# yahoo0742/COSNet

Measured on AMD Instinct MI355X. Metric: frame-pairs/sec (fwd+bwd) at 473x473 RGBD, higher is better.
Workload: dtype bf16; 1 GPU; RGBDSegmentation_RAA train step (fwd+loss+bwd+SGD), 473x473, batch 4 pairs/GPU; model=RGBDSegmentation_RAA(Bottleneck,[3,4,23,3],[3,4,6,3],1), global_batch=4, parallelism=dp1

## Files before the change

### cosnet_amd/_native.py

```python
import ctypes
import os

import torch

_HERE = os.path.dirname(os.path.abspath(__file__))
LIB_PATH = os.environ.get("COSNET_HIP_LIB") or os.path.join(_HERE, "_lib", "libcosnet_hip.so")

DT_F32 = 0
DT_BF16 = 1

_P = ctypes.c_void_p
_I = ctypes.c_int
_L = ctypes.c_longlong
_F = ctypes.c_float
_S = ctypes.c_size_t

_SIGS = {
    "cn_conv_fwd": (_I, [_I, _P, _L, _I, _I, _I, _I, _P, _I, _I, _I, _I, _I, _I, _P, _P, _L, _I, _I, _P]),
    "cn_conv_fwd_ws": (_I, [_I, _P, _L, _I, _I, _I, _I, _P, _I, _I, _I, _I, _I, _I, _P, _P, _L, _I, _I,
                            _P, _S, _P]),
    "cn_conv_fwd_workspace_floats": (_S, [_I, _I, _I, _I]),
    "cn_conv_dgrad": (_I, [_I, _P, _L, _I, _I, _I, _I, _P, _I, _I, _I, _I, _I, _I, _P, _L, _I, _I, _I, _P]),
    "cn_conv_wgrad_workspace_floats": (_S, [_I, _I, _I, _I, _I, _I, _I, _I]),
    "cn_conv_wgrad": (_I, [_I, _P, _L, _I, _I, _I, _I, _P, _L, _I, _I, _I, _I, _I, _I, _I, _I, _P, _P, _P]),
# ... 66 lines not shown
    "cn_avgpool": (_I, [_I, _P, _L, _I, _I, _I, _F, _P, _P, _P]),
    "cn_avgpool_workspace_floats": (_S, [_I, _I, _I, _I]),
    "cn_bcast_rows": (_I, [_I, _P, _I, _I, _I, _F, _P, _L, _I, _P]),
    "cn_gate_fwd": (_I, [_I, _P, _L, _I, _I, _P, _P, _P, _L, _P, _P]),
    "cn_gate_bwd": (_I, [_I, _P, _L, _P, _L, _P, _I, _I, _P, _I, _P, _L, _P, _P, _P, _P]),
    "cn_colpart_workspace_floats": (_S, [_I, _I]),
    "cn_mean_rows": (_I, [_P, _I, _I, _P, _P]),
    "cn_sum_rows": (_I, [_P, _I, _I, _P, _P]),
    "cn_scale_dev": (_I, [_P, _L, _P, _P, _P]),
    "cn_scale": (_I, [_P, _L, _F, _P]),
    "cn_soft_iou": (_I, [_P, _P, _I, _L, _P, _P, _P, _P]),
    "cn_frame_resize": (_I, [_I, _P, _I, _L, _L, _L, _I, _I, _I, _I, _P, _P, _I, _I, _I, _I, _P]),
    "cn_gemm_force_config": (_I, [_I]),
    "cn_gemm_ws_mode": (_I, [_I]),
    "cn_gemm_ws_launches": (_S, []),
    "cn_gemm_set_wgrad_target": (_I, [_I]),
    "cn_coatt_force_variant": (_I, [_I]),
    "cn_head_fwd": (_I, [_I, _P, _L, _P, _L, _I, _I, _I, _P, _P, _P, _L, _P, _P]),
    "cn_head_bwd": (_I, [_I, _P, _L, _P, _I, _I, _I, _P, _P, _L, _P, _P, _P, _P]),
    "cn_upsample_sigmoid": (_I, [_P, _I, _I, _I, _I, _I, _I, _P, _P]),
    "cn_upsample_sigmoid_bwd": (_I, [_P, _P, _I, _I, _I, _I, _I, _I, _P, _P]),
    "cn_count_ge": (_I, [_P, _L, _F, _P, _P]),
    "cn_loss_workspace_floats": (_S, [_L]),
    "cn_bce_l1": (_I, [_P, _P, _L, _F, _F, _P, _P, _P, _P]),
    "cn_bce_l1_devcount": (_I, [_P, _P, _L, _P, ctypes.c_double, _F, _P, _P, _P, _P]),
    "cn_sgd": (_I, [_P, _I, _P, _F, _F, _P]),
    "cn_rowdot": (_I, [_I, _P, _L, _P, _L, _I, _I, _P, _P]),
    "cn_colsum": (_I, [_I, _P, _L, _I, _I, _P, _P, _P]),
    "cn_cast2d": (_I, [_I, _I, _P, _L, _I, _I, _P, _L, _I, _P]),
    "cn_build_source_hash": (ctypes.c_char_p, []),
# ... 17 lines not shown
    if not os.path.exists(LIB_PATH):
        raise NativeError("libcosnet_hip.so not built (%s); run __graft_entry__.build()" % LIB_PATH)
    lib = ctypes.CDLL(LIB_PATH, mode=ctypes.RTLD_GLOBAL)
    for name, (res, args) in _SIGS.items():
        if os.environ.get("COSNET_HIP_LIB") and not hasattr(lib, name):
            continue
        fn = getattr(lib, name)
        fn.restype = res
        fn.argtypes = args
    _lib = lib
    return lib


HASHED_SOURCES = ["gemm.hip", "gemm_ws.hip", "conv.hip", "bn.hip", "ew.hip", "coatt.hip", "coatt_fused.hip",
                  "coatt_q48.hip", "coatt_flash.hip", "coatt_f8.hip", "fp8.hip", "frames.hip", "eval.hip",
                  "common.h", "gemm.h", "gemm_dev.h", "coatt_fused.h", "../../include/cosnet_hip.h"]


def source_hash():
    import hashlib
    h = hashlib.sha256()
    for f in HASHED_SOURCES:
        with open(os.path.join(_HERE, "csrc", f), "rb") as fh:
            h.update(fh.read())
    return h.hexdigest()[:16]


def build_info():
    import hashlib
    lib_hash = load().cn_build_source_hash().decode()
    with open(LIB_PATH, "rb") as fh:
# ... 39 lines not shown
```

### cosnet_amd/csrc/bn.hip

```cpp
#include "common.h"
#include "../../include/cosnet_hip.h"

namespace {

constexpr int UNR = 4;
constexpr int SUNR = 8;

struct Layout {
  int CPR, CB, RPB;
};
template <class T> __host__ __device__ inline Layout layout_red(int C) {
  Layout l;
  l.CPR = C / VecOf<T>::N;
  l.CB = l.CPR < 32 ? l.CPR : 32;
  l.RPB = 256 / l.CB;
  return l;
}
template <class T> __host__ __device__ inline Layout layout_of(int C) {
  Layout l;
  l.CPR = C / VecOf<T>::N;
  l.CB = l.CPR < 256 ? l.CPR : 256;
  l.RPB = 256 / l.CB;
  return l;
}
// ... 161 lines not shown
    const double md = s1 / n;
    const double q = s2 - s1 * md > 0 ? s2 - s1 * md : 0.0;
    const double var = q / n;
    mean[seg * C + c] = (float)(K + md);
    invstd[seg * C + c] = (float)(1.0 / sqrt(var + (double)eps));
    if (run_mean) {
      const double unb = n > 1 ? q / (n - 1) : var;
      rm = (float)((1.0 - momentum) * rm + momentum * (K + md));
      rv = (float)((1.0 - momentum) * rv + momentum * unb);
    }
  }
  if (run_mean) { run_mean[c] = (float)rm; run_var[c] = (float)rv; }
}

template <int NSEG>
__global__ __launch_bounds__(256) void bn_tile_stats_finalize(const float* __restrict__ ws, long long plane,
                                                              int mtiles, int BM, int M, int seg_rows,
                                                              int C, float* mean, float* invstd,
                                                              float* run_mean, float* run_var,
                                                              float momentum, float eps) {
  const int c0 = blockIdx.x * FCH;
  const int ch = threadIdx.x % FCH, lane = threadIdx.x / FCH, c = c0 + ch;
  double d1[NSEG], d2[NSEG];
#pragma unroll
  for (int s = 0; s < NSEG; ++s) { d1[s] = 0.0; d2[s] = 0.0; }
  if (c < C) {
    for (int t = lane; t < mtiles; t += 256 / FCH) {
      const int r0 = t * BM, r1 = min(M, r0 + BM);
      const int sA = r0 / seg_rows;
      const int endA = min(r1, (sA + 1) * seg_rows);
      const double nA = endA - r0, nB = r1 - endA;
      const long long o = (long long)t * C + c;
      const double K = ws[o];
      const double a1 = ws[o + plane], a2 = ws[o + 2 * plane];
#pragma unroll
      for (int s = 0; s < NSEG; ++s) {
        if (s == sA) { d1[s] += nA * K + a1; d2[s] += a2 + 2.0 * K * a1 + nA * K * K; }
        if (s == sA + 1 && nB > 0) {
          const double b1 = ws[o + 3 * plane], b2 = ws[o + 4 * plane];
          d1[s] += nB * K + b1;
          d2[s] += b2 + 2.0 * K * b1 + nB * K * K;
        }
      }
    }
  }
  __shared__ double red[2 * NSEG][4][FCH];
  const int wave = threadIdx.x / 64;
#pragma unroll
  for (int s = 0; s < NSEG; ++s) {
#pragma unroll
    for (int o = FCH; o < 64; o <<= 1) {
      d1[s] += __shfl_xor(d1[s], o, 64);
      d2[s] += __shfl_xor(d2[s], o, 64);
    }
    if ((threadIdx.x & 63) < FCH) { red[2 * s][wave][ch] = d1[s]; red[2 * s + 1][wave][ch] = d2[s]; }
  }
  __syncthreads();
  if (threadIdx.x >= FCH || c >= C) return;
  double rm = 0, rv = 0;
  if (run_mean) { rm = run_mean[c]; rv = run_var[c]; }
// ... 1 lines not shown
  for (int s = 0; s < NSEG; ++s) {
    const double s1 = ((red[2 * s][0][ch] + red[2 * s][1][ch]) + red[2 * s][2][ch]) + red[2 * s][3][ch];
    const double s2 = ((red[2 * s + 1][0][ch] + red[2 * s + 1][1][ch]) + red[2 * s + 1][2][ch]) + red[2 * s + 1][3][ch];
    const double md = s1 / n;
    double var = s2 / n - md * md;
    if (var < 0) var = 0;
    mean[s * C + c] = (float)md;
    invstd[s * C + c] = (float)(1.0 / sqrt(var + (double)eps));
    if (run_mean) {
      const double unb = n > 1 ? var * n / (n - 1) : var;
      rm = (float)((1.0 - momentum) * rm + momentum * md);
      rv = (float)((1.0 - momentum) * rv + momentum * unb);
    }
  }
  if (run_mean) { run_mean[c] = (float)rm; run_var[c] = (float)rv; }
}

__global__ void bn_eval_params(const float* rm, const float* rv, int C, float eps, float* mean, float* invstd) {
  int c = blockIdx.x * blockDim.x + threadIdx.x;
  if (c >= C) return;
  mean[c] = rm[c];
  invstd[c] = 1.0f / sqrtf(rv[c] + eps);
}

__device__ __forceinline__ unsigned pack4_fp8_bn(float a, float b, float c, float d) {
  a = fminf(fmaxf(a, -448.f), 448.f);
  b = fminf(fmaxf(b, -448.f), 448.f);
  c = fminf(fmaxf(c, -448.f), 448.f);
  d = fminf(fmaxf(d, -448.f), 448.f);
  unsigned w = __builtin_amdgcn_cvt_pk_fp8_f32(a, b, 0, false);
// ... 390 lines not shown
  const int seg_rows = M / nseg;
  const dim3 fin((C + FCH - 1) / FCH);
#define CN_TF(NS)                                                                                    \
  hipLaunchKernelGGL((bn_tile_stats_finalize<NS>), fin, dim3(256), 0, st, ws, plane, mtiles, BM, M, \
                     seg_rows, C, mean, invstd, run_mean, run_var, momentum, eps)
  switch (nseg) {
    case 1: CN_TF(1); break;
    case 2: CN_TF(2); break;
    default: return CN_ERR_UNSUPPORTED;
  }
#undef CN_TF
  CN_CHECK_LAUNCH();
  return 0;
}

int cn_bn_tile_bwd_impl(const float* ws, int mtiles, int C, float* sum_dz, float* sum_dzxh,
                        hipStream_t st) {
  const dim3 fin((C + FCH - 1) / FCH);
  hipLaunchKernelGGL(bn_bwd_finalize<2>, fin, dim3(256), 0, st, ws, mtiles, C, sum_dz, sum_dzxh,
                     (float*)nullptr);
  CN_CHECK_LAUNCH();
  return 0;
}

extern "C" int cn_bn_bwd_apply(int dtype, const void* x, long long ldx, const void* dy, long long lddy,
                               int P, int C, const float* mean, const float* invstd,
                               const float* gamma, const float* beta, const float* sum_dz,
                               const float* sum_dzxh, void* dx, long long lddx, hipStream_t st) {
  return with_dtype(dtype, [&](auto tag) {
    using T = tag_t<decltype(tag)>;
// ... 135 lines not shown
```

### cosnet_amd/csrc/conv.hip

```cpp
#include "gemm.h"
#include "../../include/cosnet_hip.h"

static GemmArgs gemm_defaults() {
  GemmArgs a = {};
  a.nsplit = 1;
  a.k_chunk = 1 << 30;
  a.alpha = 1.f;
  a.cfg = -1;
  FastDiv one = fastdiv_make(1);
  a.ga.div_C = a.ga.div_KW = a.ga.div_OW = a.ga.div_OHW = one;
  a.gb = a.ga;
  a.rm_div_OW = a.rm_div_OHW = one;
  return a;
}

static ConvGeom make_geom(int N, int H, int W, int C, int OH, int OW, int KH, int KW, int st,
                          int off_y, int off_x, int step_y, int step_x) {
  ConvGeom g;
  g.N = N; g.H = H; g.W = W; g.C = C; g.OH = OH; g.OW = OW; g.KH = KH; g.KW = KW; g.st = st;
  g.off_y = off_y; g.off_x = off_x; g.step_y = step_y; g.step_x = step_x;
  g.div_C = fastdiv_make(C);
  g.div_KW = fastdiv_make(KW);
  g.div_OW = fastdiv_make(OW);
  g.div_OHW = fastdiv_make(OH * OW);
// ... 193 lines not shown
  if (!fp8_operands_ok(Cout, lddy, dy8, wt8)) return CN_ERR_ALIGN;
  if (lddx % 8 || misaligned(dx)) return CN_ERR_ALIGN;
  GemmArgs a;
  int la;
  int rc = conv_dgrad_args(dy8, lddy, N, OH, OW, Cout, wt8, Cin, KH, KW, pad, dil, dx, lddx, H, W,
                           accumulate, true, a, la);
  if (rc) return rc;
  a.scale_a = dy_state;
  a.scale_b = w_state;
  return cn_gemm_dispatch(a, DT_FP8_E5M2, 0, la, L_KC_DENSE, 1, st);
}

int cn_bn_tile_stats_impl(const float* ws, long long plane, int mtiles, int BM, int M, int nseg, int C,
                          float* mean, float* invstd, float* run_mean, float* run_var, float momentum,
                          float eps, hipStream_t st);
int cn_bn_tile_bwd_impl(const float* ws, int mtiles, int C, float* sum_dz, float* sum_dzxh,
                        hipStream_t st);

static long long mtiles_of(int dtype, int M, int N, int K) {
  const int bm = cn_gemm_bm(dtype, M, N, K, -1);
  return (M + bm - 1) / bm;
}

extern "C" size_t cn_conv_fwd_bn_workspace_floats(int dtype, int M, int Cout, int K) {
  return (size_t)5 * mtiles_of(dtype, M, Cout, K) * Cout;
}

static int gemm_bn_stats(GemmArgs& a, int dtype, int la, int G, int nseg, float* const* ws,
                         float* const* mean, float* const* invstd, float* const* run_mean,
                         float* const* run_var, float momentum, float eps, hipStream_t st) {
  const int bm = cn_gemm_bm(dtype, a.M, a.N, a.K, -1);
  const long long mt = (a.M + bm - 1) / bm;
  a.st_mode = 1;
  a.st_ws = ws[0];
  a.st_plane = mt * a.N;
  a.st_seg_rows = a.M / nseg;
  int rc = cn_gemm_dispatch(a, dtype, 0, la, L_KC_DENSE, G, st);
  for (int g = 0; g < G && !rc; ++g)
    rc = cn_bn_tile_stats_impl(ws[g], a.st_plane, (int)mt, bm, a.M, nseg, a.N, mean[g], invstd[g],
                               run_mean[g], run_var[g], momentum, eps, st);
  return rc;
}

extern "C" int cn_conv_fwd_bn(int dtype, const void* x, long long ldx, int N, int H, int W, int Cin,
                              const void* w, int Cout, int KH, int KW, int stride, int pad, int dil,
                              const float* bias, void* y, long long ldy, int OH, int OW, int nseg,
                              float* ws, float* mean, float* invstd, float* run_mean, float* run_var,
                              float momentum, float eps, hipStream_t st) {
  GemmArgs a;
  int la;
  int rc = conv_fwd_args(dtype, x, ldx, N, H, W, Cin, w, Cout, KH, KW, stride, pad, dil, bias, y,
// ... 369 lines not shown
```

### cosnet_amd/csrc/gemm.h

```cpp
#pragma once
#include "common.h"

enum LoadKind { L_KC_DENSE = 0, L_KC_CONV = 1, L_MC_DENSE = 2, L_MC_CONV = 3,
                L_KC_CONV_G = 4 };

struct ConvGeom {
  int N, H, W, C;
  int OH, OW;
  int KH, KW;
  int st;
  int off_y, off_x, step_y, step_x;
  FastDiv div_C, div_KW, div_OW, div_OHW;
};

constexpr int GEMM_MAXG = 24;
struct GemmGroup {
  const void* A[GEMM_MAXG];
  const void* B[GEMM_MAXG];
  void* C[GEMM_MAXG];
  const float* SA[GEMM_MAXG];
  const float* SB[GEMM_MAXG];
  const float* bias[GEMM_MAXG];
  float* ST[GEMM_MAXG];
  int dil[GEMM_MAXG];
// ... 22 lines not shown
  long long st_plane;
  int st_seg_rows;
  const void* br_x; long long br_ldx;
  const float* br_mean; const float* br_invstd; const float* br_gamma; const float* br_beta;
  int ngroup;
  GemmGroup grp;
  int wt;
};

int cn_gemm_dispatch(const GemmArgs& a, int dtype, int c_f32, int la, int lb, int batch, hipStream_t st);
int cn_gemm_pick(int M, int N, int K, int batch_splits);
long long cn_gemm_cfg_blocks(int cfg, int M, int N);
int cn_gemm_bm(int dtype, int M, int N, int K, int cfg_or_minus1);
bool cn_gemm_ws_supports(const GemmArgs& a);
int cn_gemm_ws_launch(const GemmArgs& a, int walkers_per_xcd, hipStream_t st);
int cn_splitk_reduce_impl(const float* ws, int nsplit, long long slab, long long n, float* out,
                          int accumulate, hipStream_t st);
```

### cosnet_amd/csrc/gemm.hip

```cpp
#include "common.h"
#include "gemm.h"
#include "gemm_dev.h"
#include "../../include/cosnet_hip.h"

#include <type_traits>

namespace {

template <class T> struct Frag;
template <> struct Frag<bf16> { typedef bf16x8 type; };
template <> struct Frag<float> { typedef f32x4 type; };

__device__ __forceinline__ int mc_swz(int k, int granules_per_row) {
  int h = (k & 3) | (((k >> 3) & 1) << 2);
  return (granules_per_row >= 32 ? h : (h & 3)) << 2;
}

__device__ __forceinline__ int mc_swz8(int k) { return (k & 7) ^ ((k >> 5) & 1); }

__device__ __attribute__((aligned(16))) unsigned g_zero16[4];

__device__ __forceinline__ void glds16(const void* src, char* lds_wave_base) {
  __builtin_amdgcn_global_load_lds((const __attribute__((address_space(1))) void*)src,
                                   (__attribute__((address_space(3))) void*)lds_wave_base, 16, 0, 0);
// ... 1013 lines not shown
  return launch_c<f8e5m2, float, 11, L_MC_DENSE, LB>(a, batch, st);
}

static bool buf_ok(int kind, const GemmArgs& a, bool is_a, int esz) {
  const long long ld = is_a ? a.lda : a.ldb;
  const ConvGeom& g = is_a ? a.ga : a.gb;
  const long long kspan = a.nsplit > 1 ? a.k_chunk : a.K;
  if (kind == L_KC_DENSE) return 256 * ld * esz < 0x80000000ll && (long long)a.K * esz < 0xFFFF0000ll;
  if (kind == L_KC_CONV) return (long long)g.N * g.H * g.W * ld * esz < 0x80000000ll;
  if (kind == L_MC_DENSE) return (kspan + 128) * ld * esz < 0xFFFF0000ll && 128 * ld * esz < 0x80000000ll;
  return true;
}

static int g_ws_mode = 1;
static size_t g_ws_launches = 0;
static bool ws_heuristic(const GemmArgs& a) {
  return a.K <= 256 && a.N >= 4 * a.K && a.M >= 8192;
}
static bool ws_eligible(const GemmArgs& a, int dtype, int c_f32, int la, int lb, int batch) {
  if (!g_ws_mode || g_force_cfg >= 0 || a.cfg >= 0) return false;
  if (dtype != DT_BF16 || c_f32 || la != L_KC_DENSE || lb != L_KC_DENSE) return false;
  if (batch != 1 || a.nsplit != 1 || a.row_map || a.ngroup || a.st_mode) return false;
  if ((a.c_mode != 0 && a.c_mode != 2) || a.bias || a.alpha != 1.f || a.scale_a || a.scale_b) return false;
  if (!cn_gemm_ws_supports(a)) return false;
  return g_ws_mode >= 2 || ws_heuristic(a);
}

int cn_gemm_dispatch(const GemmArgs& a_in, int dtype, int c_f32, int la, int lb, int batch, hipStream_t st) {
  GemmArgs a = a_in;
  a.wt = a.c_mode != 1 && a.c_mode != 3 ? 4 : 0;
  if (a.M <= 0 || a.N <= 0 || batch <= 0) return 0;
  const int esz = (dtype == DT_FP8 || dtype == DT_FP8_E5M2) ? 1 : dtype == DT_BF16 ? 2 : 4;
  const int bk = 128 / esz;
  if (la == L_KC_CONV && (a.ga.C % bk != 0 || !buf_ok(L_KC_CONV, a, true, esz))) la = L_KC_CONV_G;
  if (!buf_ok(la, a, true, esz) || !buf_ok(lb, a, false, esz)) return CN_ERR_SHAPE;
  if (ws_eligible(a, dtype, c_f32, la, lb, batch)) {
    ++g_ws_launches;
    return cn_gemm_ws_launch(a, g_ws_mode == 3 ? 1 : 0, st);
  }
  if (dtype == DT_FP8) {
// ... 136 lines not shown
```

### cosnet_amd/csrc/gemm_ws.hip

```cpp
#include "common.h"
#include "gemm.h"
#include "gemm_dev.h"
#include "../../include/cosnet_hip.h"

#include <algorithm>
#include <cstdlib>
#include <type_traits>

namespace {

struct WsArgs {
  int M, N;
  const bf16* A; long long lda;
  const bf16* B; long long ldb;
  bf16* C; long long ldc;
  int nslices;
  int wpx;
  int wt;
};

__device__ __forceinline__ u32x4 load16_asm(const void* p) {
  u32x4 v;
  asm volatile("global_load_dwordx4 %0, %1, off" : "=&v"(v) : "v"(p) : "memory");
  return v;
}

template <int KEEP, bool TIE, int N>
__device__ __forceinline__ void wait_keep(u32x4 (&x)[N]) {
  static_assert(KEEP < 64, "vmcnt is 6 bits");
  asm volatile("s_waitcnt vmcnt(%0)" :: "n"(KEEP) : "memory");
  if constexpr (TIE) {
#pragma unroll
    for (int i = 0; i < N; ++i) asm volatile("" : "+v"(x[i]));
  }
}

template <int KT, int BM, int BN, int WM, int WN, bool MODE2, bool BREG>
__global__ __launch_bounds__(WM * WN * 64, 1) void gemm_ws_kernel(WsArgs p) {
  constexpr int NT = WM * WN * 64;
  constexpr int BBYTES = KT * BN * 128, ASTG = KT * BM * 128;
  constexpr int TM = BM / WM, TN = BN / WN;
  constexpr int RM = TM / 16, RN = TN / 16;
  constexpr int NCA = BM * 8 / NT, NCB = BN * 8 / NT;
  constexpr int RSTEP = NT / 8;
  constexpr int CSB = TM * TN * 4;
  constexpr int GPR = TN / 8, RPP = 64 / GPR, IT = TM / RPP;
  static_assert(NCA >= 1 && NCA * NT == BM * 8 && NCB * NT == BN * 8, "tiles fill whole chunk rounds");
  static_assert(RSTEP % 8 == 0, "a thread's chunks share row & 7");
  static_assert(IT >= 1 && IT * RPP == TM && (RN & (RN - 1)) == 0, "epilogue passes");
  static_assert(BBYTES + 2 * ASTG + WM * WN * CSB <= 160 * 1024, "LDS budget");
  __shared__ __attribute__((aligned(16))) char smem[BBYTES + 2 * ASTG + WM * WN * CSB];

  const int tid = threadIdx.x, lane = tid & 63;
  const int wave = __builtin_amdgcn_readfirstlane(tid >> 6);
  const int wm = wave / WN, wn = wave % WN;

  const int xcd = blockIdx.x & 7, j = blockIdx.x >> 3;
  const int slice = j % p.nslices;
  const int walker = xcd * p.wpx + j / p.nslices, nwalk = 8 * p.wpx;
  const int n0 = slice * BN;
  const int m16 = (p.M + 15) >> 4;
  const int r0 = (int)((long long)m16 * walker / nwalk) * 16;
  const int r1 = min(p.M, (int)((long long)m16 * (walker + 1) / nwalk) * 16);
  if (r0 >= r1) return;
  const int ntiles = (r1 - r0 + BM - 1) / BM;

  char* Bs = smem;
  char* As = smem + BBYTES;
  float* cs = (float*)(smem + BBYTES + 2 * ASTG + wave * CSB);
  const int wbase = __builtin_amdgcn_readfirstlane((tid & ~63) * 16);

  const int kcol = ((tid & 7) ^ ((tid >> 3) & 7)) * 8;
  const int rl0 = tid >> 3;

  {
    const __amdgpu_buffer_rsrc_t rb = buf_rsrc(p.B + (long long)n0 * p.ldb);
#pragma unroll
    for (int i = 0; i < NCB; ++i) {
// ... 30 lines not shown
  if constexpr (MODE2) fetch_c(0);
  wait_keep<0, MODE2>(xnx);
  raw_barrier();

  bf16x8 breg[BREG ? KT * 2 : 1][RN];
  if constexpr (BREG) {
#pragma unroll
    for (int kt = 0; kt < KT; ++kt)
#pragma unroll
      for (int pc = 0; pc < 2; ++pc)
#pragma unroll
        for (int jj = 0; jj < RN; ++jj)
          breg[kt * 2 + pc][jj] = read_frag_kc_bf16(Bs + kt * BN * 128, wn * TN + jj * 16, pc, lane);
  }

  auto epilogue = [&](int t, auto aux_c, const f32x4 (&acc)[RM][RN]) {
    constexpr int AUX = decltype(aux_c)::value;
    const int m0 = r0 + t * BM;
    const __amdgpu_buffer_rsrc_t rc = buf_rsrc(p.C + (long long)m0 * p.ldc);
    const int g = lane >> 4;
#pragma unroll
    for (int i = 0; i < RM; ++i)
#pragma unroll
      for (int jj = 0; jj < RN; ++jj)
#pragma unroll
        for (int r = 0; r < 4; ++r)
          cs[(i * 16 + 4 * g + r) * TN + (((jj ^ (g & (RN - 1))) << 4) | (lane & 15))] = acc[i][jj][r];
    asm volatile("s_waitcnt lgkmcnt(0)" ::: "memory");
#pragma unroll
    for (int it = 0; it < IT; ++it) {
      const int rr = lane / GPR + it * RPP;
      const int c0 = ((lane % GPR) * 8) ^ ((((rr >> 2) & 3) & (RN - 1)) << 4);
      float v[8];
      *(f32x4*)&v[0] = *(const f32x4*)&cs[rr * TN + c0];
      *(f32x4*)&v[4] = *(const f32x4*)&cs[rr * TN + c0 + 4];
      if constexpr (MODE2) {
        float q[8];
        Chunk<bf16>::unpack(xpf[it], q);
#pragma unroll
        for (int e = 0; e < 8; ++e) v[e] += q[e];
      }
      const int row = erow + it * RPP;
      const unsigned off = (m0 + row < r1 && col_ok) ? (unsigned)(((long long)row * p.ldc + ecol) * 2) : BUF_OOB;
      __builtin_amdgcn_raw_buffer_store_b128(Chunk<bf16>::pack(v), rc, (int)off, 0, AUX);
    }
    asm volatile("" ::: "memory");
  };

#pragma unroll 1
  for (int t = 0; t < ntiles; ++t) {
    char* cur = As + (t & 1) * ASTG;
    if constexpr (MODE2) {
#pragma unroll
      for (int it = 0; it < IT; ++it) xpf[it] = xnx[it];
    }
    if (t + 1 < ntiles) {
      issue_a(t + 1, As + ((t + 1) & 1) * ASTG);
      if constexpr (MODE2) fetch_c(t + 1);
    }
// ... 16 lines not shown
        }
#pragma unroll
        for (int i = 0; i < RM; ++i)
#pragma unroll
          for (int jj = 0; jj < RN; ++jj)
            acc[i][jj] = __builtin_amdgcn_mfma_f32_16x16x32_bf16(af[i], bfr[jj], acc[i][jj], 0, 0, 0);
      }
    if (p.wt == 4) epilogue(t, std::integral_constant<int, 2>{}, acc);
    else if (p.wt) epilogue(t, std::integral_constant<int, 16>{}, acc);
    else epilogue(t, std::integral_constant<int, 0>{}, acc);
    if (t + 1 < ntiles) {
      wait_keep<IT, MODE2>(xnx);
      raw_barrier();
    }
  }
}

template <int KT, int BM, int BN, int WM, int WN, bool BREG>
int launch_ws(const GemmArgs& a, int cus, int cap, hipStream_t st) {
  WsArgs w;
  w.M = a.M; w.N = a.N;
  w.A = (const bf16*)a.A; w.lda = a.lda;
  w.B = (const bf16*)a.B; w.ldb = a.ldb;
  w.C = (bf16*)a.C; w.ldc = a.ldc;
  w.nslices = (a.N + BN - 1) / BN;
  w.wt = a.wt;
  const int per_xcd = cus / 8;
  const int want = (int)((((long long)a.M + 15) / 16 + 7) / 8);
  w.wpx = std::min(per_xcd / w.nslices, std::max(want, 1));
  if (cap > 0) w.wpx = std::min(w.wpx, cap);
  if (w.wpx < 1) return CN_ERR_UNSUPPORTED;
  const dim3 grid(8 * w.wpx * w.nslices), block(WM * WN * 64);
  if (a.c_mode == 2)
    hipLaunchKernelGGL((gemm_ws_kernel<KT, BM, BN, WM, WN, true, BREG>), grid, block, 0, st, w);
  else
    hipLaunchKernelGGL((gemm_ws_kernel<KT, BM, BN, WM, WN, false, BREG>), grid, block, 0, st, w);
  CN_CHECK_LAUNCH();
  return 0;
}

int device_cus() {
  static const int n = [] {
    int dev = 0, v = 0;
    if (hipGetDevice(&dev) != hipSuccess) return 0;
    if (hipDeviceGetAttribute(&v, hipDeviceAttributeMultiprocessorCount, dev) != hipSuccess) return 0;
    return v;
  }();
  return n;
// ... 6 lines not shown
bool cn_gemm_ws_supports(const GemmArgs& a) {
  if (a.K != 64 && a.K != 128 && a.K != 256 && a.K != 512) return false;
  if (a.ka_lim < a.K || a.kb_lim < a.K) return false;
  if (a.N % 8 || a.ldc % 8 || (uintptr_t)a.C % 16) return false;
  if (a.lda % 8 || a.ldb % 8 || (uintptr_t)a.A % 16 || (uintptr_t)a.B % 16) return false;
  if (256 * a.ldc * 2 >= 0x80000000ll) return false;
  const int cus = device_cus();
  return cus >= 8 && (a.N + ws_bn(a.K) - 1) / ws_bn(a.K) <= cus / 8;
}

int cn_gemm_ws_launch(const GemmArgs& a, int walkers_per_xcd, hipStream_t st) {
  const int cus = device_cus();
  switch (a.K) {
    case 64:
      if (a.c_mode == 2) return launch_ws<1, 64, 128, 2, 2, true>(a, cus, walkers_per_xcd, st);
      return launch_ws<1, 128, 128, 4, 2, true>(a, cus, walkers_per_xcd, st);
    case 128: return launch_ws<2, 128, 128, 4, 2, true>(a, cus, walkers_per_xcd, st);
    case 256: return launch_ws<4, 64, 128, 2, 4, true>(a, cus, walkers_per_xcd, st);
    case 512: return launch_ws<8, 32, 64, 2, 2, false>(a, cus, walkers_per_xcd, st);
    default: return CN_ERR_UNSUPPORTED;
  }
}
```

### cosnet_amd/encoder_fn.py

```python
import os

import torch

from . import _native as nv
from . import ops
from .fp8 import fp8_ok
from .ops import WCACHE, as_param_grad, bn_apply, bn_bwd, bn_stats, conv_dgrad, conv_fwd, conv_wgrad

from .functions import F, _GRAD


class GradSink(dict):

    def __init__(self, arena=None):
        super().__init__()
        self.arena = arena

    def buf(self, p, *shape):
        if self.arena is None or p not in self.arena:
            return None
        return self.arena[p].view(*shape)

    def __setitem__(self, p, g):
        if self.arena is not None and p in self.arena:
# ... 78 lines not shown
    def __init__(self, stats, nseg, c):
        self.mean, self.invstd = stats
        self.nseg, self.c = nseg, c

    def __len__(self):
        return self.nseg

    def __getitem__(self, i):
        return ops.seg_of((self.mean, self.invstd), i, self.c)


def seg_stats(x, bn, training, nseg):
    return SegStats(bn_stats(x, bn, training, nseg=nseg), nseg, x.shape[1])


def fuse_stats(cout, kdim):
    return kdim >= 1024 and cout <= 512


def fuse_bwd(cin, kdim):
    return kdim >= 1024 and cin <= 256


def conv_bn(x, n, h, w, wf, cout, k, stride, pad, dil, bn, training, nseg, bias=None, weight=None,
            q8=None):
    cin = wf.shape[1] // (k * k)
    ctx = fp8_of(bn)
    if weight is not None and ctx is not None and fp8_ok(x, cin) and x.shape[0] > 64:
        x8, xs = ctx.acts.quant(x, id(weight))
        if q8 is not None:
            q8.append(ctx.acts.saved(x8, xs))
        wf8, ws = ctx.weights.get(weight)
        if training and FP8_FUSE_STATS and fuse_stats(cout, wf.shape[1]):
            c, oh, ow, st = ops.conv_fwd_fp8_bn(x8, n, h, w, wf8, cout, k, stride, pad, dil, xs, ws,
                                                bn, nseg, bias=bias)
            return c, oh, ow, SegStats(st, nseg, cout)
        c, oh, ow = ops.conv_fwd_fp8(x8, n, h, w, wf8, cout, k, stride, pad, dil, xs, ws, bias=bias)
        return c, oh, ow, seg_stats(c, bn, training, nseg)
    if training and fuse_stats(cout, wf.shape[1]):
        c, oh, ow, st = ops.conv_fwd_bn(x, n, h, w, wf, cout, k, stride, pad, dil, bn, nseg, bias=bias)
        return c, oh, ow, SegStats(st, nseg, cout)
    c, oh, ow = conv_fwd(x, n, h, w, wf, cout, k, stride, pad, dil, bias=bias)
    return c, oh, ow, seg_stats(c, bn, training, nseg)


def seg_apply(x, stats, bn, act=0, prelu=None, res=None, xr=None, rstats=None, rbn=None, out=None,
              fp8_key=None, mask=None):
    rs = None if rstats is None else (rstats.mean, rstats.invstd)
    ctx = fp8_of(bn)
    if fp8_key is None or ctx is None or x.dtype != torch.bfloat16:
        return bn_apply(x, (stats.mean, stats.invstd), bn, act=act, prelu=prelu, res=res, xr=xr,
                        rstats=rs, rbn=rbn, out=out, nseg=stats.nseg, mask=mask)
    st = ctx.acts.ready(fp8_key, x.device)
    if st is None:
# ... 418 lines not shown
```

### include/cosnet_hip.h

```cpp
#ifndef COSNET_HIP_H
#define COSNET_HIP_H
#include <stddef.h>
#include <hip/hip_runtime_api.h>

#ifdef __cplusplus
extern "C" {
#endif

#define CN_ERR_SHAPE (-1)
#define CN_ERR_ALIGN (-2)
#define CN_ERR_UNSUPPORTED (-3)
#define CN_ERR_HIP (-4)


int cn_conv_fwd(int dtype, const void* x, long long ldx, int N, int H, int W, int Cin,
                const void* w, int Cout, int KH, int KW, int stride, int pad, int dil,
                const float* bias, void* y, long long ldy, int OH, int OW, hipStream_t stream);

size_t cn_conv_fwd_workspace_floats(int dtype, int M, int Cout, int K);
int cn_conv_fwd_ws(int dtype, const void* x, long long ldx, int N, int H, int W, int Cin,
                   const void* w, int Cout, int KH, int KW, int stride, int pad, int dil,
                   const float* bias, void* y, long long ldy, int OH, int OW, float* ws,
                   size_t ws_floats, hipStream_t stream);

// ... 224 lines not shown
                  int seg, int seg_ld, float* out, hipStream_t stream);
int cn_colsum(int dtype, const void* x, long long ld, int P, int C, float* out,
              float* ws , hipStream_t stream);
int cn_cast2d(int dtype_in, int dtype_out, const void* x, long long ldx, int P, int C, void* y,
              long long ldy, int accumulate, hipStream_t stream);
int cn_frame_resize(int src_u8, const void* src, int C, long long plane_stride, long long row_stride,
                    long long col_stride, int y0, int x0, int h, int w, const float* mean,
                    float* dst, int H, int W, int mode, int flip, hipStream_t stream);

const char* cn_build_source_hash(void);
int cn_build_experimental(void);

int cn_gemm_force_config(int cfg);
int cn_gemm_ws_mode(int mode);
size_t cn_gemm_ws_launches(void);
int cn_gemm_set_wgrad_target(int blocks);
int cn_coatt_force_variant(int v);

#ifdef __cplusplus
}
#endif
#endif
```

Measured before the change: 137.1 frame-pairs/s.

## Fuse BN batch statistics into walker-scheduled 1x1 conv GEMM epilogue

Extends the walker-scheduled (work-stealing style) bf16 GEMM kernel with a STATS variant that accumulates per-column shifted sums and sums of squares, split by segment, in its epilogue. It reduces them via DPP and LDS into per-walker double partials, and a new finalize kernel turns those into BN mean/invstd. Plain 1x1 convs that match the walker heuristic (small K, large M) now route through this fused path instead of a separate stats pass over the output. The cost is extra epilogue arithmetic and register pressure in the GEMM, plus a larger workspace.

```diff
diff --git a/cosnet_amd/_native.py b/cosnet_amd/_native.py
--- a/cosnet_amd/_native.py
+++ b/cosnet_amd/_native.py
@@ -104,6 +104,7 @@
     "cn_gemm_force_config": (_I, [_I]),
     "cn_gemm_ws_mode": (_I, [_I]),
     "cn_gemm_ws_launches": (_S, []),
+    "cn_gemm_ws_bn_default": (_I, [_I, _I, _I]),
     "cn_gemm_set_wgrad_target": (_I, [_I]),
     "cn_coatt_force_variant": (_I, [_I]),
     "cn_head_fwd": (_I, [_I, _P, _L, _P, _L, _I, _I, _I, _P, _P, _P, _L, _P, _P]),
@@ -151,7 +152,7 @@
 
 HASHED_SOURCES = ["gemm.hip", "gemm_ws.hip", "conv.hip", "bn.hip", "ew.hip", "coatt.hip", "coatt_fused.hip",
                   "coatt_q48.hip", "coatt_flash.hip", "coatt_f8.hip", "fp8.hip", "frames.hip", "eval.hip",
-                  "common.h", "gemm.h", "gemm_dev.h", "coatt_fused.h", "../../include/cosnet_hip.h"]
+                  "common.h", "gemm.h", "gemm_dev.h", "ws_walk.h", "coatt_fused.h", "../../include/cosnet_hip.h"]
 
 
 def source_hash():
diff --git a/cosnet_amd/csrc/bn.hip b/cosnet_amd/csrc/bn.hip
--- a/cosnet_amd/csrc/bn.hip
+++ b/cosnet_amd/csrc/bn.hip
@@ -1,4 +1,5 @@
 #include "common.h"
+#include "ws_walk.h"
 #include "../../include/cosnet_hip.h"
 
 namespace {
@@ -199,36 +200,11 @@
 }
 
 template <int NSEG>
-__global__ __launch_bounds__(256) void bn_tile_stats_finalize(const float* __restrict__ ws, long long plane,
-                                                              int mtiles, int BM, int M, int seg_rows,
-                                                              int C, float* mean, float* invstd,
-                                                              float* run_mean, float* run_var,
-                                                              float momentum, float eps) {
-  const int c0 = blockIdx.x * FCH;
-  const int ch = threadIdx.x % FCH, lane = threadIdx.x / FCH, c = c0 + ch;
-  double d1[NSEG], d2[NSEG];
-#pragma unroll
-  for (int s = 0; s < NSEG; ++s) { d1[s] = 0.0; d2[s] = 0.0; }
-  if (c < C) {
-    for (int t = lane; t < mtiles; t += 256 / FCH) {
-      const int r0 = t * BM, r1 = min(M, r0 + BM);
-      const int sA = r0 / seg_rows;
-      const int endA = min(r1, (sA + 1) * seg_rows);
-      const double nA = endA - r0, nB = r1 - endA;
-      const long long o = (long long)t * C + c;
-      const double K = ws[o];
-      const double a1 = ws[o + plane], a2 = ws[o + 2 * plane];
-#pragma unroll
-      for (int s = 0; s < NSEG; ++s) {
-        if (s == sA) { d1[s] += nA * K + a1; d2[s] += a2 + 2.0 * K * a1 + nA * K * K; }
-        if (s == sA + 1 && nB > 0) {
-          const double b1 = ws[o + 3 * plane], b2 = ws[o + 4 * plane];
-          d1[s] += nB * K + b1;
-          d2[s] += b2 + 2.0 * K * b1 + nB * K * K;
-        }
-      }
-    }
-  }
+__device__ __forceinline__ void seg_sums_finish(double (&d1)[NSEG], double (&d2)[NSEG], int c, int C,
+                                                int seg_rows, float* mean, float* invstd,
+                                                float* run_mean, float* run_var, float momentum,
+                                                float eps) {
+  const int ch = threadIdx.x % FCH;
   __shared__ double red[2 * NSEG][4][FCH];
   const int wave = threadIdx.x / 64;
 #pragma unroll
@@ -260,6 +236,64 @@
     }
   }
   if (run_mean) { run_mean[c] = (float)rm; run_var[c] = (float)rv; }
+}
+
+template <int NSEG>
+__global__ __launch_bounds__(256) void bn_tile_stats_finalize(const float* __restrict__ ws, long long plane,
+                                                              int mtiles, int BM, int M, int seg_rows,
+                                                              int C, float* mean, float* invstd,
+                                                              float* run_mean, float* run_var,
+                                                              float momentum, float eps) {
+  const int c0 = blockIdx.x * FCH;
+  const int ch = threadIdx.x % FCH, lane = threadIdx.x / FCH, c = c0 + ch;
+  double d1[NSEG], d2[NSEG];
+#pragma unroll
+  for (int s = 0; s < NSEG; ++s) { d1[s] = 0.0; d2[s] = 0.0; }
+  if (c < C) {
+    for (int t = lane; t < mtiles; t += 256 / FCH) {
+      const int r0 = t * BM, r1 = min(M, r0 + BM);
+      const int sA = r0 / seg_rows;
+      const int endA = min(r1, (sA + 1) * seg_rows);
+      const double nA = endA - r0, nB = r1 - endA;
+      const long long o = (long long)t * C + c;
+      const double K = ws[o];
+      const double a1 = ws[o + plane], a2 = ws[o + 2 * plane];
+#pragma unroll
+      for (int s = 0; s < NSEG; ++s) {
+        if (s == sA) { d1[s] += nA * K + a1; d2[s] += a2 + 2.0 * K * a1 + nA * K * K; }
+        if (s == sA + 1 && nB > 0) {
+          const double b1 = ws[o + 3 * plane], b2 = ws[o + 4 * plane];
+          d1[s] += nB * K + b1;
+          d2[s] += b2 + 2.0 * K * b1 + nB * K * K;
+        }
+      }
+    }
+  }
+  seg_sums_finish<NSEG>(d1, d2, c, C, seg_rows, mean, invstd, run_mean, run_var, momentum, eps);
+}
+
+template <int NSEG>
+__global__ __launch_bounds__(256) void bn_walk_stats_finalize(const double* __restrict__ ws, int nwalk,
+                                                              int M, int seg_rows, int C, float* mean,
+                                                              float* invstd, float* run_mean,
+                                                              float* run_var, float momentum, float eps) {
+  const int c = blockIdx.x * FCH + threadIdx.x % FCH, lane = threadIdx.x / FCH;
+  double d1[NSEG], d2[NSEG];
+#pragma unroll
+  for (int s = 0; s < NSEG; ++s) { d1[s] = 0.0; d2[s] = 0.0; }
+  if (c < C) {
+    for (int w = lane; w < nwalk; w += 256 / FCH) {
+      const WsRows r = ws_walker_rows(M, w, nwalk);
+      if (r.r0 >= r.r1) continue;
+      const double* o = ws + (long long)w * WS_ST_PLANES * C + c;
+#pragma unroll
+      for (int s = 0; s < NSEG; ++s) {
+        d1[s] += o[(long long)(2 * s) * C];
+        d2[s] += o[(long long)(2 * s + 1) * C];
+      }
+    }
+  }
+  seg_sums_finish<NSEG>(d1, d2, c, C, seg_rows, mean, invstd, run_mean, run_var, momentum, eps);
 }
 
 __global__ void bn_eval_params(const float* rm, const float* rv, int C, float eps, float* mean, float* invstd) {
@@ -680,6 +714,24 @@
   return 0;
 }
 
+int cn_bn_walk_stats_impl(const float* ws, int nwalk, int M, int nseg, int C, float* mean, float* invstd,
+                          float* run_mean, float* run_var, float momentum, float eps, hipStream_t st) {
+  if (nseg < 1 || M % nseg || nwalk < 1 || (uintptr_t)ws % 8) return CN_ERR_SHAPE;
+  const int seg_rows = M / nseg;
+  const dim3 fin((C + FCH - 1) / FCH);
+#define CN_WF(NS)                                                                                     \
+  hipLaunchKernelGGL((bn_walk_stats_finalize<NS>), fin, dim3(256), 0, st, (const double*)ws, nwalk, M, \
+                     seg_rows, C, mean, invstd, run_mean, run_var, momentum, eps)
+  switch (nseg) {
+    case 1: CN_WF(1); break;
+    case 2: CN_WF(2); break;
+    default: return CN_ERR_UNSUPPORTED;
+  }
+#undef CN_WF
+  CN_CHECK_LAUNCH();
+  return 0;
+}
+
 int cn_bn_tile_bwd_impl(const float* ws, int mtiles, int C, float* sum_dz, float* sum_dzxh,
                         hipStream_t st) {
   const dim3 fin((C + FCH - 1) / FCH);
diff --git a/cosnet_amd/csrc/conv.hip b/cosnet_amd/csrc/conv.hip
--- a/cosnet_amd/csrc/conv.hip
+++ b/cosnet_amd/csrc/conv.hip
@@ -231,6 +231,8 @@
 int cn_bn_tile_stats_impl(const float* ws, long long plane, int mtiles, int BM, int M, int nseg, int C,
                           float* mean, float* invstd, float* run_mean, float* run_var, float momentum,
                           float eps, hipStream_t st);
+int cn_bn_walk_stats_impl(const float* ws, int nwalk, int M, int nseg, int C, float* mean, float* invstd,
+                          float* run_mean, float* run_var, float momentum, float eps, hipStream_t st);
 int cn_bn_tile_bwd_impl(const float* ws, int mtiles, int C, float* sum_dz, float* sum_dzxh,
                         hipStream_t st);
 
@@ -240,7 +242,9 @@
 }
 
 extern "C" size_t cn_conv_fwd_bn_workspace_floats(int dtype, int M, int Cout, int K) {
-  return (size_t)5 * mtiles_of(dtype, M, Cout, K) * Cout;
+  const size_t tiles = (size_t)5 * mtiles_of(dtype, M, Cout, K) * Cout;
+  const size_t walk = cn_gemm_ws_bn_floats(dtype, M, Cout, K);
+  return tiles > walk ? tiles : walk;
 }
 
 static int gemm_bn_stats(GemmArgs& a, int dtype, int la, int G, int nseg, float* const* ws,
@@ -252,6 +256,13 @@
   a.st_ws = ws[0];
   a.st_plane = mt * a.N;
   a.st_seg_rows = a.M / nseg;
+  const int nwalk = cn_gemm_bn_route(a, dtype, la, G);
+  if (nwalk > 0) {
+    const int rc = cn_gemm_dispatch(a, dtype, 0, la, L_KC_DENSE, G, st);
+    return rc ? rc : cn_bn_walk_stats_impl(ws[0], nwalk, a.M, nseg, a.N, mean[0], invstd[0], run_mean[0],
+                                           run_var[0], momentum, eps, st);
+  }
+  if (dtype == DT_BF16) a.cfg = cn_gemm_pick(a.M, a.N, a.K, 1);
   int rc = cn_gemm_dispatch(a, dtype, 0, la, L_KC_DENSE, G, st);
   for (int g = 0; g < G && !rc; ++g)
     rc = cn_bn_tile_stats_impl(ws[g], a.st_plane, (int)mt, bm, a.M, nseg, a.N, mean[g], invstd[g],
diff --git a/cosnet_amd/csrc/gemm.h b/cosnet_amd/csrc/gemm.h
--- a/cosnet_amd/csrc/gemm.h
+++ b/cosnet_amd/csrc/gemm.h
@@ -60,5 +60,8 @@
 int cn_gemm_bm(int dtype, int M, int N, int K, int cfg_or_minus1);
 bool cn_gemm_ws_supports(const GemmArgs& a);
 int cn_gemm_ws_launch(const GemmArgs& a, int walkers_per_xcd, hipStream_t st);
+int cn_gemm_ws_walkers(int M, int N, int K, int walkers_per_xcd);
+int cn_gemm_bn_route(const GemmArgs& a, int dtype, int la, int batch);
+size_t cn_gemm_ws_bn_floats(int dtype, int M, int N, int K);
 int cn_splitk_reduce_impl(const float* ws, int nsplit, long long slab, long long n, float* out,
                           int accumulate, hipStream_t st);
diff --git a/cosnet_amd/csrc/gemm.hip b/cosnet_amd/csrc/gemm.hip
--- a/cosnet_amd/csrc/gemm.hip
+++ b/cosnet_amd/csrc/gemm.hip
@@ -1,6 +1,7 @@
 #include "common.h"
 #include "gemm.h"
 #include "gemm_dev.h"
+#include "ws_walk.h"
 #include "../../include/cosnet_hip.h"
 
 #include <type_traits>
@@ -1051,16 +1052,33 @@
 
 static int g_ws_mode = 1;
 static size_t g_ws_launches = 0;
-static bool ws_heuristic(const GemmArgs& a) {
-  return a.K <= 256 && a.N >= 4 * a.K && a.M >= 8192;
+static bool ws_heuristic(int M, int N, int K) {
+  return K <= 256 && N >= 4 * K && M >= 8192;
 }
 static bool ws_eligible(const GemmArgs& a, int dtype, int c_f32, int la, int lb, int batch) {
   if (!g_ws_mode || g_force_cfg >= 0 || a.cfg >= 0) return false;
   if (dtype != DT_BF16 || c_f32 || la != L_KC_DENSE || lb != L_KC_DENSE) return false;
-  if (batch != 1 || a.nsplit != 1 || a.row_map || a.ngroup || a.st_mode) return false;
+  if (batch != 1 || a.nsplit != 1 || a.row_map || a.ngroup) return false;
   if ((a.c_mode != 0 && a.c_mode != 2) || a.bias || a.alpha != 1.f || a.scale_a || a.scale_b) return false;
+  if (a.st_mode && (a.st_mode != 1 || a.c_mode != 0 || a.K > 256 || !a.st_ws || (uintptr_t)a.st_ws % 8 ||
+                    a.st_seg_rows < 1 || 2ll * a.st_seg_rows < a.M))
+    return false;
   if (!cn_gemm_ws_supports(a)) return false;
-  return g_ws_mode >= 2 || ws_heuristic(a);
+  return g_ws_mode >= 2 || ws_heuristic(a.M, a.N, a.K);
+}
+
+int cn_gemm_bn_route(const GemmArgs& a, int dtype, int la, int batch) {
+  if (a.st_mode != 1 || !ws_eligible(a, dtype, 0, la, L_KC_DENSE, batch)) return 0;
+  return cn_gemm_ws_walkers(a.M, a.N, a.K, g_ws_mode == 3 ? 1 : 0);
+}
+
+size_t cn_gemm_ws_bn_floats(int dtype, int M, int N, int K) {
+  if (dtype != DT_BF16 || (K != 64 && K != 128 && K != 256) || N % 8) return 0;
+  return (size_t)2 * WS_ST_PLANES * cn_gemm_ws_walkers(M, N, K, 0) * N;
+}
+
+extern "C" int cn_gemm_ws_bn_default(int M, int N, int K) {
+  return g_ws_mode != 0 && g_force_cfg < 0 && ws_heuristic(M, N, K) && cn_gemm_ws_bn_floats(DT_BF16, M, N, K) > 0;
 }
 
 int cn_gemm_dispatch(const GemmArgs& a_in, int dtype, int c_f32, int la, int lb, int batch, hipStream_t st) {
diff --git a/cosnet_amd/csrc/gemm_ws.hip b/cosnet_amd/csrc/gemm_ws.hip
--- a/cosnet_amd/csrc/gemm_ws.hip
+++ b/cosnet_amd/csrc/gemm_ws.hip
@@ -1,6 +1,7 @@
 #include "common.h"
 #include "gemm.h"
 #include "gemm_dev.h"
+#include "ws_walk.h"
 #include "../../include/cosnet_hip.h"
 
 #include <algorithm>
@@ -17,12 +18,19 @@
   int nslices;
   int wpx;
   int wt;
+  double* st;
+  int seg_rows;
 };
 
 __device__ __forceinline__ u32x4 load16_asm(const void* p) {
   u32x4 v;
   asm volatile("global_load_dwordx4 %0, %1, off" : "=&v"(v) : "v"(p) : "memory");
   return v;
+}
+
+template <int ROR>
+__device__ __forceinline__ float row_ror(float v) {
+  return __builtin_bit_cast(float, __builtin_amdgcn_update_dpp(0, __builtin_bit_cast(int, v), 0x120 + ROR, 0xf, 0xf, false));
 }
 
 template <int KEEP, bool TIE, int N>
@@ -35,7 +43,7 @@
   }
 }
 
-template <int KT, int BM, int BN, int WM, int WN, bool MODE2, bool BREG>
+template <int KT, int BM, int BN, int WM, int WN, bool MODE2, bool BREG, bool STATS = false>
 __global__ __launch_bounds__(WM * WN * 64, 1) void gemm_ws_kernel(WsArgs p) {
   constexpr int NT = WM * WN * 64;
   constexpr int BBYTES = KT * BN * 128, ASTG = KT * BM * 128;
@@ -49,6 +57,7 @@
   static_assert(RSTEP % 8 == 0, "a thread's chunks share row & 7");
   static_assert(IT >= 1 && IT * RPP == TM && (RN & (RN - 1)) == 0, "epilogue passes");
   static_assert(BBYTES + 2 * ASTG + WM * WN * CSB <= 160 * 1024, "LDS budget");
+  static_assert(!STATS || !MODE2, "statistics: plain stores only");
   __shared__ __attribute__((aligned(16))) char smem[BBYTES + 2 * ASTG + WM * WN * CSB];
 
   const int tid = threadIdx.x, lane = tid & 63;
@@ -59,9 +68,8 @@
   const int slice = j % p.nslices;
   const int walker = xcd * p.wpx + j / p.nslices, nwalk = 8 * p.wpx;
   const int n0 = slice * BN;
-  const int m16 = (p.M + 15) >> 4;
-  const int r0 = (int)((long long)m16 * walker / nwalk) * 16;
-  const int r1 = min(p.M, (int)((long long)m16 * (walker + 1) / nwalk) * 16);
+  const WsRows wr = ws_walker_rows(p.M, walker, nwalk);
+  const int r0 = wr.r0, r1 = wr.r1;
   if (r0 >= r1) return;
   const int ntiles = (r1 - r0 + BM - 1) / BM;
 
@@ -122,6 +130,18 @@
           breg[kt * 2 + pc][jj] = read_frag_kc_bf16(Bs + kt * BN * 128, wn * TN + jj * 16, pc, lane);
   }
 
+  constexpr int SE = STATS ? 8 : 1;
+  constexpr int SPL = 5 * 8 + 2;
+  static_assert(!STATS || ((GPR == 4 || GPR == 8) && CSB >= 4 * GPR * SPL * 4 && NT == WS_ST_PLANES * BN),
+                "statistics: column groups within a DPP row; partials fit a patch; a thread per (column, plane)");
+  float sk[SE], s1[SE], s2[SE], f1[SE], f2[SE];
+  int ns = 0, nf = 0;
+  bool crossed = false;
+  if constexpr (STATS) {
+#pragma unroll
+    for (int e = 0; e < 8; ++e) sk[e] = s1[e] = s2[e] = f1[e] = f2[e] = 0.f;
+  }
+
   auto epilogue = [&](int t, auto aux_c, const f32x4 (&acc)[RM][RN]) {
     constexpr int AUX = decltype(aux_c)::value;
     const int m0 = r0 + t * BM;
@@ -135,6 +155,25 @@
         for (int r = 0; r < 4; ++r)
           cs[(i * 16 + 4 * g + r) * TN + (((jj ^ (g & (RN - 1))) << 4) | (lane & 15))] = acc[i][jj][r];
     asm volatile("s_waitcnt lgkmcnt(0)" ::: "memory");
+    bool full = false;
+    int lim = 0;
+    if constexpr (STATS) {
+      if (t == 0) {
+        float k0[8];
+        *(f32x4*)&k0[0] = *(const f32x4*)&cs[(lane % GPR) * 8];
+        *(f32x4*)&k0[4] = *(const f32x4*)&cs[(lane % GPR) * 8 + 4];
+        Chunk<bf16>::unpack(Chunk<bf16>::pack(k0), sk);
+      }
+      if (!crossed && m0 >= p.seg_rows) {
+#pragma unroll
+        for (int e = 0; e < 8; ++e) { f1[e] = s1[e]; f2[e] = s2[e]; s1[e] = 0.f; s2[e] = 0.f; }
+        nf = ns;
+        ns = 0;
+        crossed = true;
+      }
+      full = m0 + BM <= r1 && (crossed || m0 + BM <= p.seg_rows);
+      lim = crossed ? 0x7fffffff : p.seg_rows;
+    }
 #pragma unroll
     for (int it = 0; it < IT; ++it) {
       const int rr = lane / GPR + it * RPP;
@@ -150,7 +189,50 @@
       }
       const int row = erow + it * RPP;
       const unsigned off = (m0 + row < r1 && col_ok) ? (unsigned)(((long long)row * p.ldc + ecol) * 2) : BUF_OOB;
-      __builtin_amdgcn_raw_buffer_store_b128(Chunk<bf16>::pack(v), rc, (int)off, 0, AUX);
+      if constexpr (!STATS) {
+        __builtin_amdgcn_raw_buffer_store_b128(Chunk<bf16>::pack(v), rc, (int)off, 0, AUX);
+      } else {
+        const u32x4 pk = Chunk<bf16>::pack(v);
+        __builtin_amdgcn_raw_buffer_store_b128(pk, rc, (int)off, 0, AUX);
+        float q[8];
+        Chunk<bf16>::unpack(pk, q);
+        if (full) {
+#pragma unroll
+          for (int e = 0; e < 8; ++e) {
+            const float d = q[e] - sk[e];
+            s1[e] += d;
+            s2[e] = fmaf(d, d, s2[e]);
+          }
+        } else {
+          const bool ina = m0 + row < r1 && m0 + row < lim, inb = m0 + row < r1 && m0 + row >= lim;
+          const float ma = ina ? 1.f : 0.f, mb = inb ? 1.f : 0.f;
+#pragma unroll
+          for (int e = 0; e < 8; ++e) {
+            const float d = q[e] - sk[e], da = d * ma, db = d * mb;
+            s1[e] += da;
+            s2[e] = fmaf(da, da, s2[e]);
+            f1[e] += db;
+            f2[e] = fmaf(db, db, f2[e]);
+          }
+          ns += ina;
+          nf += inb;
+        }
+      }
+    }
+    if constexpr (STATS) {
+      if (full) {
+        ns += IT;
+      } else if (!crossed && m0 + BM > p.seg_rows) {
+#pragma unroll
+        for (int e = 0; e < 8; ++e) {
+          const float x1 = s1[e], x2 = s2[e];
+          s1[e] = f1[e]; s2[e] = f2[e]; f1[e] = x1; f2[e] = x2;
+        }
+        const int n = ns;
+        ns = nf;
+        nf = n;
+        crossed = true;
+      }
     }
     asm volatile("" ::: "memory");
   };
@@ -197,9 +279,57 @@
       raw_barrier();
     }
   }
-}
-
-template <int KT, int BM, int BN, int WM, int WN, bool BREG>
+
+  if constexpr (STATS) {
+    float red[SPL];
+#pragma unroll
+    for (int e = 0; e < 8; ++e) {
+      red[e] = sk[e];
+      red[8 + e] = crossed ? f1[e] : s1[e];
+      red[16 + e] = crossed ? f2[e] : s2[e];
+      red[24 + e] = crossed ? s1[e] : 0.f;
+      red[32 + e] = crossed ? s2[e] : 0.f;
+    }
+    red[40] = (float)(crossed ? nf : ns);
+    red[41] = (float)(crossed ? ns : 0);
+#pragma unroll
+    for (int v = 8; v < SPL; ++v) {
+      red[v] += row_ror<8>(red[v]);
+      if constexpr (GPR == 4) red[v] += row_ror<4>(red[v]);
+    }
+    if ((lane & 15) < GPR) {
+      float* pp = cs + ((lane >> 4) * GPR + (lane & 15)) * SPL;
+#pragma unroll
+      for (int v = 0; v < SPL; ++v) pp[v] = red[v];
+    }
+    asm volatile("s_waitcnt lgkmcnt(0)" ::: "memory");
+    raw_barrier();
+    const int col = tid % BN, q = tid / BN, sg = q >> 1;
+    const int grp = (col % TN) / 8, e = col % 8;
+    double acc = 0.0;
+#pragma unroll 1
+    for (int w = 0; w < WM; ++w) {
+      const float* pw = (const float*)(smem + BBYTES + 2 * ASTG + (w * WN + col / TN) * CSB);
+#pragma unroll
+      for (int r = 0; r < 4; ++r) {
+        const float* pp = pw + (r * GPR + grp) * SPL;
+        const double k = pp[e], n = pp[40 + sg], x1 = pp[8 + 16 * sg + e], x2 = pp[16 + 16 * sg + e];
+        acc += (q & 1) ? x2 + 2.0 * k * x1 + n * k * k : n * k + x1;
+      }
+    }
+    if (n0 + col < p.N)
+      __builtin_nontemporal_store(acc, &p.st[((long long)walker * WS_ST_PLANES + q) * p.N + n0 + col]);
+  }
+}
+
+int ws_wpx(int M, int nslices, int cus, int cap) {
+  const int want = (int)((((long long)M + 15) / 16 + 7) / 8);
+  int wpx = std::min(cus / 8 / nslices, std::max(want, 1));
+  if (cap > 0) wpx = std::min(wpx, cap);
+  return wpx;
+}
+
+template <int KT, int BM, int BN, int WM, int WN, bool BREG, bool STATS = false>
 int launch_ws(const GemmArgs& a, int cus, int cap, hipStream_t st) {
   WsArgs w;
   w.M = a.M; w.N = a.N;
@@ -208,13 +338,19 @@
   w.C = (bf16*)a.C; w.ldc = a.ldc;
   w.nslices = (a.N + BN - 1) / BN;
   w.wt = a.wt;
-  const int per_xcd = cus / 8;
-  const int want = (int)((((long long)a.M + 15) / 16 + 7) / 8);
-  w.wpx = std::min(per_xcd / w.nslices, std::max(want, 1));
-  if (cap > 0) w.wpx = std::min(w.wpx, cap);
+  w.st = (double*)a.st_ws;
+  w.seg_rows = a.st_seg_rows;
+  w.wpx = ws_wpx(a.M, w.nslices, cus, cap);
   if (w.wpx < 1) return CN_ERR_UNSUPPORTED;
   const dim3 grid(8 * w.wpx * w.nslices), block(WM * WN * 64);
-  if (a.c_mode == 2)
+  if (a.st_mode) {
+    if constexpr (STATS) {
+      if (a.st_mode != 1 || a.c_mode != 0 || !a.st_ws) return CN_ERR_UNSUPPORTED;
+      hipLaunchKernelGGL((gemm_ws_kernel<KT, BM, BN, WM, WN, false, BREG, true>), grid, block, 0, st, w);
+    } else {
+      return CN_ERR_UNSUPPORTED;
+    }
+  } else if (a.c_mode == 2)
     hipLaunchKernelGGL((gemm_ws_kernel<KT, BM, BN, WM, WN, true, BREG>), grid, block, 0, st, w);
   else
     hipLaunchKernelGGL((gemm_ws_kernel<KT, BM, BN, WM, WN, false, BREG>), grid, block, 0, st, w);
@@ -251,10 +387,16 @@
   switch (a.K) {
     case 64:
       if (a.c_mode == 2) return launch_ws<1, 64, 128, 2, 2, true>(a, cus, walkers_per_xcd, st);
-      return launch_ws<1, 128, 128, 4, 2, true>(a, cus, walkers_per_xcd, st);
-    case 128: return launch_ws<2, 128, 128, 4, 2, true>(a, cus, walkers_per_xcd, st);
-    case 256: return launch_ws<4, 64, 128, 2, 4, true>(a, cus, walkers_per_xcd, st);
+      return launch_ws<1, 128, 128, 4, 2, true, true>(a, cus, walkers_per_xcd, st);
+    case 128: return launch_ws<2, 128, 128, 4, 2, true, true>(a, cus, walkers_per_xcd, st);
+    case 256: return launch_ws<4, 64, 128, 2, 4, true, true>(a, cus, walkers_per_xcd, st);
     case 512: return launch_ws<8, 32, 64, 2, 2, false>(a, cus, walkers_per_xcd, st);
     default: return CN_ERR_UNSUPPORTED;
   }
 }
+
+int cn_gemm_ws_walkers(int M, int N, int K, int walkers_per_xcd) {
+  const int nslices = (N + ws_bn(K) - 1) / ws_bn(K);
+  const int wpx = ws_wpx(M, nslices, device_cus(), walkers_per_xcd);
+  return wpx < 1 ? 0 : 8 * wpx;
+}
diff --git a/cosnet_amd/csrc/ws_walk.h b/cosnet_amd/csrc/ws_walk.h
--- /dev/null
+++ b/cosnet_amd/csrc/ws_walk.h
@@ -0,0 +1,16 @@
+#pragma once
+
+struct WsRows {
+  int r0, r1;
+};
+
+__host__ __device__ inline WsRows ws_walker_rows(int M, int walker, int nwalk) {
+  const int m16 = (M + 15) >> 4;
+  WsRows r;
+  r.r0 = (int)((long long)m16 * walker / nwalk) * 16;
+  const int e = (int)((long long)m16 * (walker + 1) / nwalk) * 16;
+  r.r1 = M < e ? M : e;
+  return r;
+}
+
+constexpr int WS_ST_PLANES = 4;
diff --git a/cosnet_amd/encoder_fn.py b/cosnet_amd/encoder_fn.py
--- a/cosnet_amd/encoder_fn.py
+++ b/cosnet_amd/encoder_fn.py
@@ -116,8 +116,10 @@
     return SegStats(bn_stats(x, bn, training, nseg=nseg), nseg, x.shape[1])
 
 
-def fuse_stats(cout, kdim):
-    return kdim >= 1024 and cout <= 512
+def fuse_stats(cout, kdim, rows=0, plain_1x1=False):
+    if kdim >= 1024 and cout <= 512:
+        return True
+    return plain_1x1 and bool(nv.query("cn_gemm_ws_bn_default", rows, cout, kdim))
 
 
 def fuse_bwd(cin, kdim):
@@ -139,7 +141,8 @@
             return c, oh, ow, SegStats(st, nseg, cout)
         c, oh, ow = ops.conv_fwd_fp8(x8, n, h, w, wf8, cout, k, stride, pad, dil, xs, ws, bias=bias)
         return c, oh, ow, seg_stats(c, bn, training, nseg)
-    if training and fuse_stats(cout, wf.shape[1]):
+    plain_1x1 = x.dtype == torch.bfloat16 and k == 1 and stride == 1 and pad == 0 and bias is None
+    if training and fuse_stats(cout, wf.shape[1], x.shape[0], plain_1x1):
         c, oh, ow, st = ops.conv_fwd_bn(x, n, h, w, wf, cout, k, stride, pad, dil, bn, nseg, bias=bias)
         return c, oh, ow, SegStats(st, nseg, cout)
     c, oh, ow = conv_fwd(x, n, h, w, wf, cout, k, stride, pad, dil, bias=bias)
diff --git a/include/cosnet_hip.h b/include/cosnet_hip.h
--- a/include/cosnet_hip.h
+++ b/include/cosnet_hip.h
@@ -262,6 +262,7 @@
 int cn_gemm_force_config(int cfg);
 int cn_gemm_ws_mode(int mode);
 size_t cn_gemm_ws_launches(void);
+int cn_gemm_ws_bn_default(int M, int N, int K);
 int cn_gemm_set_wgrad_target(int blocks);
 int cn_coatt_force_variant(int v);
 
```

Result: no change. 138.0 frame-pairs/s, median of 6 (+0.7%).
